# grantjr1842/delayed-streams-modeling

Measured on AMD Instinct MI355X. Metric: real-time stream throughput, stt-1b-en_fr @ bs=64 per GPU (Mimi encode + LM decode per 80 ms frame), higher is better.
Workload: dtype bf16 weights + bf16 KV, f32 activations as three exact bf16 pieces, f32 accumulate (v_mfma_f32_16x16x32_bf16); 1 GPU; stt-1b-en_fr batch=64 streaming, ring KV cache full (750 frames), Mimi encode + LM decode HIP path; streams_per_gpu=64, parallelism=replicas x1 (independent stream batches, no per-step collective), streams=encoder stream || 2 LM group stream(s)

## Files before the change

delayed-streams-modeling_amd/csrc/dsm_device.h:

```cpp
#pragma once
#include <hip/hip_runtime.h>

#include <atomic>
#include <cstdarg>
#include <cstdio>
#include <cstdlib>
#include <deque>
#include <mutex>
#include <shared_mutex>
#include <string>
#include <vector>

#include "../../include/dsm.h"
#include "dsm_gemm_plan.h"

#define HIPCHK_E(eng, expr)                                                                         \
  do {                                                                                              \
    hipError_t _e = (expr);                                                                         \
    if (_e != hipSuccess) {                                                                         \
      (eng)->set_error("%s failed: %s (%s:%d)", #expr, hipGetErrorString(_e), __FILE__, __LINE__);  \
      return DSM_ERR_DEVICE;                                                                        \
    }                                                                                               \
  } while (0)
#define HIPCHK(expr) HIPCHK_E(e, expr)

static void dsm_read_env(struct DsmDevice* e, bool stt);

struct DsmDevice {
  int device = 0;
  bool opened = false;
  hipStream_t s_enc = nullptr, s_model = nullptr;
  static constexpr int kMaxGroups = 4;
  hipStream_t s_grp[kMaxGroups] = {nullptr, nullptr, nullptr, nullptr};
  hipEvent_t ev_fork = nullptr, ev_grp_done[kMaxGroups] = {};
  bool prio_streams = false;
  int prio_hi = 0;
  bool use_graphs = true;
  bool fuse_qkv = true;
  bool stream_prio = false;
  bool fuse_front = true;
  int chunk_loop_min_tiles = GemmKnobs().chunk_loop_min_tiles;
  int loop_depth = GemmKnobs().loop_depth;
  int smallk_min_tiles = GemmKnobs().smallk_min_tiles;
  int smallk_mt = GemmKnobs().smallk_mt;
  size_t attn_lds_pad = 60000;
  int dot_mode = 0;

  int open(int device_id, int dot_mode_, bool stt) {
    device = device_id;
    dot_mode = dot_mode_;
    int ndev = 0;
    if (hipGetDeviceCount(&ndev) != hipSuccess || ndev <= device_id) {
      set_error("no usable HIP device %d (found %d): libdsm_mi355x has no CPU fallback", device_id, ndev);
      return DSM_ERR_DEVICE;
    }
    HIPCHK_E(this, hipSetDevice(device_id));
    opened = true;
    dsm_read_env(this, stt);
    prio_streams = stt;
    int prio_lo = 0;
    if (stt && stream_prio) (void)hipDeviceGetStreamPriorityRange(&prio_lo, &prio_hi);
    if (int rc = new_stream(&s_enc, prio_lo)) return rc;
    return new_stream(&s_model, prio_hi);
  }
  int new_stream(hipStream_t* out, int prio) {
    HIPCHK_E(this, prio_streams ? hipStreamCreateWithPriority(out, hipStreamNonBlocking, prio)
                                : hipStreamCreateWithFlags(out, hipStreamNonBlocking));
    return 0;
  }
  int open_groups(int G) {
    for (int g = 1; g < G; ++g) {
      if (int rc = new_stream(&s_grp[g], prio_hi)) return rc;
      if (int rc = new_event(&ev_grp_done[g])) return rc;
// ... 246 lines not shown
```

delayed-streams-modeling_amd/csrc/dsm_engine.hip:

```cpp
#include <hip/hip_runtime.h>

#include <cmath>
#include <cstdarg>
#include <cstdio>
#include <cstdlib>
#include <cstring>
#include <atomic>
#include <map>
#include <mutex>
#include <shared_mutex>
#include <string>
#include <set>
#include <vector>

#include "../../include/dsm.h"
#include "dsm_device.h"
#include "dsm_config_presets.h"
#include "dsm_gemm_plan.h"
#include "dsm_kernels.h"
#include "dsm_pcm_table.inc"
#include "dsm_numerics.h"
#include "dsm_safetensors.h"
#include "dsm_slot_blob.h"
#include "dsm_tts_slot_blob.h"
#include "dsm_tts_slot_layout.h"
#include "dsm_spm.h"
#include "dsm_slot_xfer.inc"
#include "dsm_asr_clip.h"

static thread_local std::string g_create_error;

static int dsm_env_int(const char* name, int dflt) {
  const char* v = getenv(name);
  return v ? atoi(v) : dflt;
}
static void dsm_read_env(DsmDevice* e, bool stt) {
  e->chunk_loop_min_tiles = gemm_default_knobs(stt, e->dot_mode).chunk_loop_min_tiles;
  if (stt && e->dot_mode == 1) e->attn_lds_pad = 40000;
  e->use_graphs = dsm_env_int("DSM_GRAPHS", 1) != 0;
  e->fuse_qkv = dsm_env_int("DSM_FUSE_QKV", 1) != 0;
  e->stream_prio = dsm_env_int("DSM_STREAM_PRIO", 0) != 0;
  e->fuse_front = dsm_env_int("DSM_FUSE_FRONT", 1) != 0;
  e->chunk_loop_min_tiles = dsm_env_int("DSM_CHUNK_LOOP_MIN", e->chunk_loop_min_tiles);
  e->loop_depth = dsm_env_int("DSM_LOOP_DEPTH", e->loop_depth) == 2 ? 2 : 4;
  e->smallk_min_tiles = dsm_env_int("DSM_SMALLK_MIN", e->smallk_min_tiles);
  const int mt = dsm_env_int("DSM_SMALLK_MT", e->smallk_mt);
  if (mt == 1 || mt == 2 || mt == 4) e->smallk_mt = mt;
}


namespace {

struct Linear {
  void* w = nullptr;
  float* bias = nullptr;
  int N = 0, K = 0, Npad = 0, Kpad = 0;
  bool bf16 = false;
  bool packed = false;
};

struct ConvGeom {
  Linear lin;
  int in_c = 0, out_c = 0, k = 0, stride = 1;
  int S = 0;
  int T_in = 0;
  int T_out = 0;
  bool replicate = false;
};

ConvGeom over_frames(const ConvGeom& g, int r) {
  ConvGeom c = g;
  c.T_in *= r;
  c.T_out *= r;
  return c;
}
// ... 1031 lines not shown
```

delayed-streams-modeling_amd/csrc/dsm_engine_api.inc:

```

namespace {

template <typename KVT, int HD, int T>
int launch_attn_t(DsmDevice* e, hipStream_t st, float* out, const float* q, const void* k, const void* v,
                  const uint32_t* start_pos, const uint8_t* active, int B, int H, int ctx, int d, const AttnFused& fq) {
  constexpr int UNR = (sizeof(KVT) == 2 && T == 1 && HD == 128) ? 8 : 4;
  size_t lds = sizeof(float) * ((size_t)T * ctx + 4 * T * HD + 16);
  if ((long)B * H >= 2048 && (size_t)2 * ctx * HD * sizeof(KVT) >= (size_t)256 * 1024) lds += e->attn_lds_pad;
  if (lds > 64 * 1024) {
    static size_t allowed = 0;
    if (lds > allowed) {
      HIPCHK(hipFuncSetAttribute(reinterpret_cast<const void*>(&attn_kernel<KVT, HD, T, UNR>), hipFuncAttributeMaxDynamicSharedMemorySize, (int)lds));
      allowed = lds;
    }
  }
  const int tag = e->tag_attn[e->sid(st)];
  if (T == 1 && HD == 64 && ctx <= 32) {
    const int ph = e->prof_begin(tag, st);
    hipLaunchKernelGGL((attn_small_kernel<KVT, 64>), dim3((B * H + 3) / 4), dim3(256), 0, st, out, q, reinterpret_cast<const KVT*>(k),
                       reinterpret_cast<const KVT*>(v), start_pos, active, B * H, H, ctx, d, fq);
    e->prof_end(ph, st);
    HIPCHK(hipGetLastError());
    return 0;
  }
// ... 123 lines not shown
    if (phase == 1) return 0;
    if (int rc = transformer_layer_tail<WT, KVT>(e, st, w, l, act, B, T, final_out, final_map, post_norm_w, post_norm_out, ca)) return rc;
  }
  return 0;
}

template <typename F>
int with_kv_type(bool kv_bf16, F&& f) {
  return kv_bf16 ? f(uint16_t{}) : f(float{});
}

int fork_groups(DsmDevice* e, hipStream_t st, size_t G) {
  if (G > 1) {
    HIPCHK(hipEventRecord(e->ev_fork, st));
    for (size_t g = 1; g < G; ++g) HIPCHK(hipStreamWaitEvent(e->s_grp[g], e->ev_fork, 0));
  }
  return 0;
}
template <typename F>
int run_groups(DsmDevice* e, hipStream_t st, size_t G, bool serialize, F&& body) {
  for (size_t g = G; g-- > 0;) {
    hipStream_t gs = (g == 0 || serialize) ? st : e->s_grp[g];
    if (int rc = body(g, gs)) return rc;
    if (g > 0) HIPCHK(hipEventRecord(e->ev_grp_done[g], gs));
  }
  return 0;
}
int join_groups(DsmDevice* e, hipStream_t st, size_t G) {
  for (size_t g = 1; g < G; ++g) HIPCHK(hipStreamWaitEvent(st, e->ev_grp_done[g], 0));
  return 0;
}

int seanet_encode(DsmDevice* e, hipStream_t st, const MimiW& w, SeanetEnc& s, const float* cat_init, int B, int r, float* out,
                  RowMap omap, bool front_done = false) {
  const RowMap none = plain_map(1, 1);
  const size_t n = w.stages.size();
  const ConvGeom g0 = over_frames(w.init_conv, r), gf = over_frames(w.final_conv, r);
  if (!front_done)
    if (int rc = run_conv(e, st, g0, cat_init, B, s.stages[0].y, plain_map(B * g0.T_out, g0.out_c), s.stages[0].cat_ra,
                          cat_map(over_frames(w.stages[0].ra, r)), nullptr, none))
      return rc;
  for (size_t i = 0; i < n; ++i) {
    const ConvGeom ra = over_frames(w.stages[i].ra, r), rb = over_frames(w.stages[i].rb, r), dn = over_frames(w.stages[i].down, r);
    SeanetEnc::Stage& ss = s.stages[i];
    if (!(i == 0 && front_done)) {
      if (int rc = run_conv(e, st, ra, ss.cat_ra, B, nullptr, none, ss.cat_rb, cat_map(rb), nullptr, none)) return rc;
      if (int rc = run_conv(e, st, rb, ss.cat_rb, B, nullptr, none, ss.cat_down, cat_map(dn), ss.y, plain_map(B * rb.T_out, rb.out_c)))
        return rc;
    }
    if (i + 1 < n) {
      if (int rc = run_conv(e, st, dn, ss.cat_down, B, s.stages[i + 1].y, plain_map(B * dn.T_out, dn.out_c), s.stages[i + 1].cat_ra,
                            cat_map(over_frames(w.stages[i + 1].ra, r)), nullptr, none))
        return rc;
    } else if (int rc = run_conv(e, st, dn, ss.cat_down, B, nullptr, none, s.cat_final, cat_map(gf), nullptr, none)) {
      return rc;
    }
  }
  return run_conv(e, st, gf, s.cat_final, B, out, omap, nullptr, none, nullptr, none);
}

int mimi_encode_body(dsm_engine* e, int side, hipStream_t st);
int mimi_encode(dsm_engine* e, int side, hipStream_t st) {
  return run_captured(e, *e->g_enc[side], st, (uint64_t)e->sid(st), [&] { return mimi_encode_body(e, side, st); });
}
int mimi_encode_body(dsm_engine* e, int side, hipStream_t st) {
  const MimiW& w = e->mimi_w;
  MimiState& s = e->mimi[side];
  const int B = e->B;
  const RowMap none = plain_map(1, 1);
  e->tag_gemm[e->sid(st)] = DSM_PROF_GEMM_MIMI;
  e->tag_attn[e->sid(st)] = DSM_PROF_ATTN_MIMI;
  bool fused_front = false;
  {
    const MimiW::Stage& s0 = w.stages[0];
    const ConvGeom& c = w.init_conv;
    fused_front = e->fuse_front && c.in_c == 1 && c.k == 7 && c.stride == 1 && c.out_c == 64 && c.S == 6 && !c.lin.bf16 &&
                  s0.ra.k == 3 && s0.ra.stride == 1 && s0.ra.in_c == 64 && s0.ra.out_c == 32 && s0.ra.S == 2 && !s0.ra.lin.bf16 &&
                  s0.rb.k == 1 && s0.rb.stride == 1 && s0.rb.in_c == 32 && s0.rb.out_c == 64 && !s0.rb.lin.bf16 &&
                  c.T_in % 64 == 0 && c.T_out == c.T_in && s0.ra.T_in == c.T_in && s0.rb.T_in == c.T_in && s0.down.in_c == 64 &&
                  s0.down.T_in == c.T_in && !c.replicate && !s0.ra.replicate;
    if (fused_front) {
      SeanetFrontArgs fa;
      fa.cat_init = s.enc.cat_init;
      fa.w0 = reinterpret_cast<const float*>(c.lin.w); fa.b0 = c.lin.bias; fa.ld0 = c.lin.Kpad;
      fa.w1 = reinterpret_cast<const float*>(s0.ra.lin.w); fa.b1 = s0.ra.lin.bias; fa.ld1 = s0.ra.lin.Kpad;
      fa.w2 = reinterpret_cast<const float*>(s0.rb.lin.w); fa.b2 = s0.rb.lin.bias; fa.ld2 = s0.rb.lin.Kpad;
      fa.cat_ra = s.enc.stages[0].cat_ra;
      fa.cat_down = s.enc.stages[0].cat_down;
      fa.T = c.T_in; fa.S0 = c.S; fa.Sd = s0.down.S;
      const int ph = e->prof_begin(e->tag_gemm[e->sid(st)], st);
      hipLaunchKernelGGL(seanet_front_kernel<64>, dim3(c.T_in / 64, B), dim3(256), seanet_front_lds<64>(), st, fa);
      e->prof_end(ph, st);
      HIPCHK(hipGetLastError());
    }
  }
  const int Tt = w.final_conv.T_out, d = w.cfg.dimension;
  if (int rc = seanet_encode(e, st, w, s.enc, s.enc.cat_init, B, 1, s.act.x, plain_map(B * Tt, d), fused_front)) return rc;
  if (int rc = transformer_forward<float, float>(e, st, w.tr, s.tr, s.act, B, Tt, s.mask, s.cat_ds, cat_map(w.downsample))) return rc;
  if (s.first_call && w.downsample.S > 0) {
    hipLaunchKernelGGL(conv_replicate_init_kernel, dim3(B), dim3(256), 0, st, s.h_descs[s.ds_desc], (const uint8_t*)s.keep);
    HIPCHK(hipGetLastError());
  }
  if (int rc = run_conv(e, st, w.downsample, s.cat_ds, B, s.latent, plain_map(B, d), nullptr, none, nullptr, none)) return rc;
  const int n_q = w.cfg.quantizer_n_q, qd = w.cfg.quantizer_dim;
  e->tag_gemm[e->sid(st)] = DSM_PROF_RVQ;
  for (int which = 0; which < 2; ++which) {
    const RvqW& r = which == 0 ? w.rvq_first : w.rvq_rest;
    if (r.n_q == 0) continue;
    float* res = which == 0 ? s.res_first : s.res_rest;
    {
      GemmArgs a = base_args(r.input_proj, s.latent, plain_map(B, d), B);
      a.Y = res; a.ymap = plain_map(B, qd);
      if (int rc = gemm_store<float>(e, st, a)) return rc;
    }
    for (int i = 0; i < r.n_q; ++i) {
      const Linear& cb = r.codebooks[i];
      GemmArgs a = base_args(cb, res, plain_map(B, qd), B);
      a.pval = s.pval; a.pidx = s.pidx;
      if (int rc = launch_gemm<float, float, EPI_RVQ, 1>(e, st, a, true)) return rc;
      hipLaunchKernelGGL(rvq_select_kernel, dim3(B), dim3(256), 0, st, s.pval, s.pidx, (cb.N + 15) / 16, B, s.codes, n_q,
                         which == 0 ? 0 : 1 + i, res, reinterpret_cast<const float*>(cb.w), qd, cb.Kpad);
      HIPCHK(hipGetLastError());
    }
  }
  if (!s.h_descs.empty()) {
    hipLaunchKernelGGL(conv_state_shift_kernel, dim3(B, (unsigned)s.h_descs.size()), dim3(256), 0, st, s.descs, s.mask,
                       s.first_call ? 1 : 0, nullptr, (const uint8_t*)(s.first_call ? s.keep : nullptr));
    HIPCHK(hipGetLastError());
  }
  s.first_call = false;
// ... 1309 lines not shown
    hipLaunchKernelGGL(fill_u32_kernel, dim3(g), dim3(256), 0, e->s_model, s.idx, pos % (uint32_t)ctx, (long)e->B);
  };
  fill(e->lm.tr, lm_pos, e->cfg.lm.context);
  for (int side = 0; side < 2; ++side)
    if (side == 0 || e->mimi1_ready.load(std::memory_order_acquire)) fill(e->mimi[side].tr, mimi_pos, e->cfg.mimi.transformer.context);
  HIPCHK(hipGetLastError());
  return dsm_sync(e);
}

int dsm_debug_set_text_tokens(dsm_engine* e, const uint32_t* tokens) {
  if (!e || !tokens) return DSM_ERR_INVALID;
  HIPCHK(hipSetDevice(e->device));
  ApiShared api(e);
  if (int rc = dsm_sync(e)) return rc;
  HIPCHK(hipMemcpy(e->lm.text_token, tokens, sizeof(uint32_t) * (size_t)e->B, hipMemcpyHostToDevice));
  return dsm_sync(e);
}

int dsm_debug_read(dsm_engine* e, const char* name, float* out, size_t cap) {
  if (!e || !name || !out) return DSM_ERR_INVALID;
  HIPCHK(hipSetDevice(e->device));
  ApiShared api(e);
  if (int rc = dsm_sync(e)) return rc;
  const float* src = nullptr;
  size_t n = 0;
  const int B = e->B, dim = e->cfg.mimi.dimension;
  int side = 0;
  std::string nm(name);
  if (nm.rfind("mimi1.", 0) == 0) { side = 1; nm = nm.substr(6); }
  else if (nm.rfind("mimi.", 0) == 0) nm = nm.substr(5);
  if (nm == "lm.hidden") { src = e->lm.hidden; n = (size_t)B * e->cfg.lm.d_model; }
  else if (nm == "lm.logits") { src = e->lm.logits; n = (size_t)B * e->cfg.text_out_vocab_size; }
  else if (nm == "latent") { src = e->mimi[side].latent; n = (size_t)B * dim; }
  if (!src) { e->set_error("unknown debug tap %s", name); return DSM_ERR_INVALID; }
  if (n > cap) n = cap;
  HIPCHK(hipMemcpy(out, src, sizeof(float) * n, hipMemcpyDeviceToHost));
  return (int)n;
}

int dsm_debug_gemm_plan(int stt, int dot_mode, int weight_bf16, int epi, int nt, int M, int N, int K, int flags, char* buf, size_t cap) {
  const int knobs[5] = {dot_mode, -1, -1, -1, -1};
  return dsm_debug_gemm_plan_knobs(stt, knobs, weight_bf16, epi, nt, M, N, K, flags, buf, cap);
}

}

namespace {
bool debug_knobs(const int* knobs, GemmKnobs* k) {
  if (knobs[0] >= 0) k->dot_mode = knobs[0];
  if (knobs[1] >= 0) k->chunk_loop_min_tiles = knobs[1];
  if (knobs[2] >= 0) k->smallk_min_tiles = knobs[2];
  if (knobs[3] >= 0) k->smallk_mt = knobs[3];
  if (knobs[4] >= 0) k->loop_depth = knobs[4];
  return (k->dot_mode == 0 || k->dot_mode == 1) && (k->smallk_mt == 1 || k->smallk_mt == 2 || k->smallk_mt == 4) &&
         (k->loop_depth == 2 || k->loop_depth == 4);
}

__global__ __launch_bounds__(256) void debug_slab_sum_kernel(float* Y, RowMap ymap, Slabs s, int M, int N) {
  const long i = (long)blockIdx.x * 256 + threadIdx.x;
  const int n4 = N >> 2;
  if (i >= (long)M * n4) return;
  const int m = (int)(i / n4), n = (int)(i % n4) * 4;
  const f32x4 v = slab_sum(s.ws + (long)m * s.ld + n, s.cstride, s.chunks);
  float* y = Y + ymap.off(m) + n;
  y[0] = v[0]; y[1] = v[1]; y[2] = v[2]; y[3] = v[3];
}
// ... 170 lines not shown
```

delayed-streams-modeling_amd/csrc/dsm_kernels.h:

```cpp
#pragma once
#include <hip/hip_runtime.h>
#include <stdint.h>
#include "dsm_numerics.h"
#include "dsm_sampling.h"
#include "dsm_token_scores.h"
#include "dsm_text_bias.h"
#include "dsm_pcm_format.h"

typedef float f32x4 __attribute__((ext_vector_type(4)));
typedef short dsm_bf16x8 __attribute__((ext_vector_type(8)));

__device__ __forceinline__ float wave_sum64(float v) {
#pragma unroll
  for (int off = 32; off >= 1; off >>= 1) v = v + __shfl_xor(v, off, 64);
  return v;
}

enum { EPI_STORE = 0, EPI_QKV = 1, EPI_GATE = 2, EPI_RVQ = 3 };

struct RowMap {
  long bstride;
  int rpb;
  int ld;
  int toff;
// ... 2139 lines not shown
      for (int i = 0; i < 4; ++i) o[i] = dsm_elu(a.b1 ? acc[m2][i] + a.b1[n + i] : acc[m2][i]);
      *reinterpret_cast<float4*>(&hs[m * C1 + 4 * ((n >> 2) ^ dsm_xs_sw(m))]) = make_float4(o[0], o[1], o[2], o[3]);
    }
  }
  __syncthreads();
  {
    f32x4 acc[MTILES];
#pragma unroll
    for (int mt = 0; mt < MTILES; ++mt) acc[mt] = (f32x4){0.f, 0.f, 0.f, 0.f};
    float wa[8], xb[MTILES][8];
    load_w8<float>(a.w2 + (long)(16 * wave + r) * a.ld2 + 8 * q, wa);
    const int xu0 = 4 * ((2 * q) ^ dsm_xs_sw(r)), xu1 = xu0 ^ 4;
#pragma unroll
    for (int mt = 0; mt < MTILES; ++mt) {
      const float* fp = &hs[(16 * mt + r) * C1];
      const float4 f0 = *reinterpret_cast<const float4*>(fp + xu0), f1 = *reinterpret_cast<const float4*>(fp + xu1);
      xb[mt][0] = f0.x; xb[mt][1] = f0.y; xb[mt][2] = f0.z; xb[mt][3] = f0.w;
      xb[mt][4] = f1.x; xb[mt][5] = f1.y; xb[mt][6] = f1.z; xb[mt][7] = f1.w;
    }
#pragma unroll
    for (int sidx = 0; sidx < 8; ++sidx)
#pragma unroll
      for (int mt = 0; mt < MTILES; ++mt) acc[mt] = __builtin_amdgcn_mfma_f32_16x16x4f32(wa[sidx], xb[mt][sidx], acc[mt], 0, 0, 0);
    float* out = a.cat_down + ((long)b * (a.Sd + a.T) + a.Sd + t0) * C0;
#pragma unroll
    for (int mt = 0; mt < MTILES; ++mt) {
      const int m = 16 * mt + r, n = 16 * wave + 4 * q;
      const float4 rv = *reinterpret_cast<const float4*>(&y0[m * C0 + 4 * ((n >> 2) ^ (m & 15))]);
      float o[4];
#pragma unroll
      for (int i = 0; i < 4; ++i) o[i] = a.b2 ? acc[mt][i] + a.b2[n + i] : acc[mt][i];
      o[0] = rv.x + o[0]; o[1] = rv.y + o[1]; o[2] = rv.z + o[2]; o[3] = rv.w + o[3];
      *reinterpret_cast<float4*>(out + (long)m * C0 + n) = make_float4(dsm_elu(o[0]), dsm_elu(o[1]), dsm_elu(o[2]), dsm_elu(o[3]));
    }
  }
}

struct ConvStateDesc {
  float* cat;
  long bstride;
  int S, T, C, replicate;
};

__global__ void conv_state_shift_kernel(const ConvStateDesc* __restrict__ descs, const uint8_t* __restrict__ active,
                                        int first_call, uint8_t* __restrict__ started, const uint8_t* __restrict__ keep) {
  const ConvStateDesc dsc = descs[blockIdx.y];
  const int b = blockIdx.x;
  float* base = dsc.cat + (long)b * dsc.bstride;
  const int n = dsc.S * dsc.C;
  if (active[b]) {
    const float* src = base + (long)dsc.T * dsc.C;
    for (int i = threadIdx.x; i < n; i += blockDim.x) base[i] = src[i];
    if (started && blockIdx.y == 0 && threadIdx.x == 0) started[b] = 1;
  } else if (first_call && !started && !(keep && keep[b])) {
    for (int i = threadIdx.x; i < n; i += blockDim.x) base[i] = 0.0f;
  }
}

__global__ void conv_replicate_init_kernel(ConvStateDesc dsc, const uint8_t* __restrict__ keep) {
  const int b = blockIdx.x;
  if (keep && keep[b]) return;
  float* base = dsc.cat + (long)b * dsc.bstride;
  const float* first = base + (long)dsc.S * dsc.C;
  for (int i = threadIdx.x; i < dsc.S * dsc.C; i += blockDim.x) base[i] = first[i % dsc.C];
}

// ... 665 lines not shown
```

Measured before the change: 1892 x realtime (stream-seconds of audio per wall second).

## Fuse SEANet stage-0 downsample and stage-1 residual block into one kernel

Adds seanet_stage1_kernel, which computes the stage-0 strided downsample conv, the stage-1 k=3 residual conv and the k=1 conv with the ELU and skip add in one launch. Each workgroup keeps a 30-frame tile plus halo in LDS and writes straight into the stage-1 down-conv input buffer. This removes three separate conv launches and the global round trips of their intermediates in the Mimi encoder. In exchange it recomputes the halo frames, depends on hard-coded channel and stride shapes guarded by a runtime check, and turns fuse_front into a tri-state so the path can be switched off.

```diff
diff --git a/delayed-streams-modeling_amd/csrc/dsm_device.h b/delayed-streams-modeling_amd/csrc/dsm_device.h
--- a/delayed-streams-modeling_amd/csrc/dsm_device.h
+++ b/delayed-streams-modeling_amd/csrc/dsm_device.h
@@ -38,7 +38,7 @@
   bool use_graphs = true;
   bool fuse_qkv = true;
   bool stream_prio = false;
-  bool fuse_front = true;
+  int fuse_front = 1;
   int chunk_loop_min_tiles = GemmKnobs().chunk_loop_min_tiles;
   int loop_depth = GemmKnobs().loop_depth;
   int smallk_min_tiles = GemmKnobs().smallk_min_tiles;
diff --git a/delayed-streams-modeling_amd/csrc/dsm_engine.hip b/delayed-streams-modeling_amd/csrc/dsm_engine.hip
--- a/delayed-streams-modeling_amd/csrc/dsm_engine.hip
+++ b/delayed-streams-modeling_amd/csrc/dsm_engine.hip
@@ -40,7 +40,8 @@
   e->use_graphs = dsm_env_int("DSM_GRAPHS", 1) != 0;
   e->fuse_qkv = dsm_env_int("DSM_FUSE_QKV", 1) != 0;
   e->stream_prio = dsm_env_int("DSM_STREAM_PRIO", 0) != 0;
-  e->fuse_front = dsm_env_int("DSM_FUSE_FRONT", 1) != 0;
+  e->fuse_front = dsm_env_int("DSM_FUSE_FRONT", 1);
+  if (e->fuse_front < 0 || e->fuse_front > 2) e->fuse_front = 1;
   e->chunk_loop_min_tiles = dsm_env_int("DSM_CHUNK_LOOP_MIN", e->chunk_loop_min_tiles);
   e->loop_depth = dsm_env_int("DSM_LOOP_DEPTH", e->loop_depth) == 2 ? 2 : 4;
   e->smallk_min_tiles = dsm_env_int("DSM_SMALLK_MIN", e->smallk_min_tiles);
diff --git a/delayed-streams-modeling_amd/csrc/dsm_engine_api.inc b/delayed-streams-modeling_amd/csrc/dsm_engine_api.inc
--- a/delayed-streams-modeling_amd/csrc/dsm_engine_api.inc
+++ b/delayed-streams-modeling_amd/csrc/dsm_engine_api.inc
@@ -179,7 +179,7 @@
 }
 
 int seanet_encode(DsmDevice* e, hipStream_t st, const MimiW& w, SeanetEnc& s, const float* cat_init, int B, int r, float* out,
-                  RowMap omap, bool front_done = false) {
+                  RowMap omap, bool front_done = false, const SeanetStage1Args* st1 = nullptr) {
   const RowMap none = plain_map(1, 1);
   const size_t n = w.stages.size();
   const ConvGeom g0 = over_frames(w.init_conv, r), gf = over_frames(w.final_conv, r);
@@ -190,12 +190,17 @@
   for (size_t i = 0; i < n; ++i) {
     const ConvGeom ra = over_frames(w.stages[i].ra, r), rb = over_frames(w.stages[i].rb, r), dn = over_frames(w.stages[i].down, r);
     SeanetEnc::Stage& ss = s.stages[i];
-    if (!(i == 0 && front_done)) {
+    if (!(i == 0 && front_done) && !(i == 1 && st1)) {
       if (int rc = run_conv(e, st, ra, ss.cat_ra, B, nullptr, none, ss.cat_rb, cat_map(rb), nullptr, none)) return rc;
       if (int rc = run_conv(e, st, rb, ss.cat_rb, B, nullptr, none, ss.cat_down, cat_map(dn), ss.y, plain_map(B * rb.T_out, rb.out_c)))
         return rc;
     }
-    if (i + 1 < n) {
+    if (i == 0 && st1) {
+      const int ph = e->prof_begin(e->tag_gemm[e->sid(st)], st);
+      hipLaunchKernelGGL(seanet_stage1_kernel, dim3(st1->T / kSeanetStage1Frames, B), dim3(256), seanet_stage1_lds(), st, *st1);
+      e->prof_end(ph, st);
+      HIPCHK(hipGetLastError());
+    } else if (i + 1 < n) {
       if (int rc = run_conv(e, st, dn, ss.cat_down, B, s.stages[i + 1].y, plain_map(B * dn.T_out, dn.out_c), s.stages[i + 1].cat_ra,
                             cat_map(over_frames(w.stages[i + 1].ra, r)), nullptr, none))
         return rc;
@@ -241,8 +246,30 @@
       HIPCHK(hipGetLastError());
     }
   }
+  SeanetStage1Args sa;
+  bool fused_stage1 = false;
+  if (e->fuse_front == 1 && w.stages.size() >= 2) {
+    const ConvGeom& dn = w.stages[0].down;
+    const MimiW::Stage& s1 = w.stages[1];
+    const int T = dn.T_out;
+    fused_stage1 = dn.in_c == 64 && dn.out_c == 128 && dn.k == 8 && dn.stride == 4 && dn.S == 4 && dn.T_in == 4 * T && !dn.lin.bf16 &&
+                   !dn.replicate && s1.ra.k == 3 && s1.ra.stride == 1 && s1.ra.in_c == 128 && s1.ra.out_c == 64 && s1.ra.S == 2 &&
+                   !s1.ra.lin.bf16 && !s1.ra.replicate && s1.rb.k == 1 && s1.rb.stride == 1 && s1.rb.in_c == 64 && s1.rb.out_c == 128 &&
+                   s1.rb.S == 0 && !s1.rb.lin.bf16 && T > 0 && T % kSeanetStage1Frames == 0 && s1.ra.T_in == T && s1.ra.T_out == T &&
+                   s1.rb.T_in == T && s1.rb.T_out == T && s1.down.in_c == 128 && s1.down.T_in == T;
+    if (fused_stage1) {
+      sa.cat_in = s.enc.stages[0].cat_down;
+      sa.wd = reinterpret_cast<const float*>(dn.lin.w); sa.bd = dn.lin.bias; sa.ldd = dn.lin.Kpad;
+      sa.w1 = reinterpret_cast<const float*>(s1.ra.lin.w); sa.b1 = s1.ra.lin.bias; sa.ld1 = s1.ra.lin.Kpad;
+      sa.w2 = reinterpret_cast<const float*>(s1.rb.lin.w); sa.b2 = s1.rb.lin.bias; sa.ld2 = s1.rb.lin.Kpad;
+      sa.cat_ra = s.enc.stages[1].cat_ra;
+      sa.cat_down = s.enc.stages[1].cat_down;
+      sa.T = T; sa.S0 = dn.S; sa.Sd = s1.down.S;
+    }
+  }
   const int Tt = w.final_conv.T_out, d = w.cfg.dimension;
-  if (int rc = seanet_encode(e, st, w, s.enc, s.enc.cat_init, B, 1, s.act.x, plain_map(B * Tt, d), fused_front)) return rc;
+  if (int rc = seanet_encode(e, st, w, s.enc, s.enc.cat_init, B, 1, s.act.x, plain_map(B * Tt, d), fused_front, fused_stage1 ? &sa : nullptr))
+    return rc;
   if (int rc = transformer_forward<float, float>(e, st, w.tr, s.tr, s.act, B, Tt, s.mask, s.cat_ds, cat_map(w.downsample))) return rc;
   if (s.first_call && w.downsample.S > 0) {
     hipLaunchKernelGGL(conv_replicate_init_kernel, dim3(B), dim3(256), 0, st, s.h_descs[s.ds_desc], (const uint8_t*)s.keep);
diff --git a/delayed-streams-modeling_amd/csrc/dsm_kernels.h b/delayed-streams-modeling_amd/csrc/dsm_kernels.h
--- a/delayed-streams-modeling_amd/csrc/dsm_kernels.h
+++ b/delayed-streams-modeling_amd/csrc/dsm_kernels.h
@@ -2195,6 +2195,229 @@
       for (int i = 0; i < 4; ++i) o[i] = a.b2 ? acc[mt][i] + a.b2[n + i] : acc[mt][i];
       o[0] = rv.x + o[0]; o[1] = rv.y + o[1]; o[2] = rv.z + o[2]; o[3] = rv.w + o[3];
       *reinterpret_cast<float4*>(out + (long)m * C0 + n) = make_float4(dsm_elu(o[0]), dsm_elu(o[1]), dsm_elu(o[2]), dsm_elu(o[3]));
+    }
+  }
+}
+
+struct SeanetStage1Args {
+  const float* cat_in;
+  const float *wd, *bd;
+  const float *w1, *b1;
+  const float *w2, *b2;
+  float* cat_ra;
+  float* cat_down;
+  int ldd, ld1, ld2;
+  int T, S0, Sd;
+};
+
+constexpr int kSeanetStage1Frames = 30;
+constexpr size_t seanet_stage1_lds() { return sizeof(float) * (132 * 64); }
+static_assert(4 * seanet_stage1_lds() <= 160 * 1024 && 34 * 128 + 32 * 64 <= 132 * 64, "four workgroups per CU; e1 and hs fit the input region");
+
+__global__ __launch_bounds__(256) void seanet_stage1_kernel(SeanetStage1Args a) {
+  constexpr int CI = 64, C1 = 128, CH = 64, TF = kSeanetStage1Frames, RIN = 4 * 32 + 4;
+  constexpr int PF = 2;
+  extern __shared__ __attribute__((aligned(16))) float st1_lds[];
+  float* xin = st1_lds;
+  float* e1 = xin;
+  float* hs = e1 + 34 * C1;
+  const int tid = threadIdx.x, lane = tid & 63, wave = tid >> 6;
+  const int r = lane & 15, q = lane >> 4;
+  const int b = blockIdx.y, t0 = blockIdx.x * TF;
+  const bool first = t0 == 0, last = t0 + TF == a.T;
+
+  const float* wrow0 = a.wd + (long)(32 * wave + r) * a.ldd + 8 * q;
+  const float* wrow1 = wrow0 + (long)16 * a.ldd;
+  float wa[PF + 1][2][8];
+#pragma unroll
+  for (int p = 0; p < PF; ++p) {
+    load_w8<float>(wrow0 + 32 * p, wa[p][0]);
+    load_w8<float>(wrow1 + 32 * p, wa[p][1]);
+  }
+  {
+    const float* src = a.cat_in + (long)b * (a.S0 + 4 * a.T) * CI;
+    constexpr int PIECES = RIN * (CI / 4), PER = (PIECES + 255) / 256;
+    float4 v[PER];
+#pragma unroll
+    for (int j = 0; j < PER; ++j) {
+      const int i = min(tid + 256 * j, PIECES - 1);
+      const int g = max(4 * (t0 - 2) + (i >> 4), 0);
+      v[j] = *reinterpret_cast<const float4*>(src + (long)g * CI + 4 * (i & 15));
+    }
+#pragma unroll
+    for (int j = 0; j < PER; ++j) {
+      const int i = tid + 256 * j, p = i >> 4;
+      if (i < PIECES) *reinterpret_cast<float4*>(&xin[p * CI + 4 * ((i & 15) ^ ((p >> 2) & 15))]) = v[j];
+    }
+  }
+  __syncthreads();
+  f32x4 y1[2][2];
+  {
+    f32x4 acc[2][2], tot[2][2];
+#pragma unroll
+    for (int blk = 0; blk < 16; ++blk) {
+      if ((blk & 7) == 0) {
+#pragma unroll
+        for (int nt = 0; nt < 2; ++nt)
+#pragma unroll
+          for (int mt = 0; mt < 2; ++mt) acc[nt][mt] = (f32x4){0.f, 0.f, 0.f, 0.f};
+      }
+      if (blk + PF < 16) {
+        load_w8<float>(wrow0 + 32 * (blk + PF), wa[(blk + PF) % (PF + 1)][0]);
+        load_w8<float>(wrow1 + 32 * (blk + PF), wa[(blk + PF) % (PF + 1)][1]);
+      }
+      const int tap = blk >> 1, u0 = (blk & 1) * 8 + 2 * q;
+      float xb[2][8];
+#pragma unroll
+      for (int mt = 0; mt < 2; ++mt) {
+        const int p = 4 * (16 * mt + r) + tap, sw = (p >> 2) & 15;
+        const float4 f0 = *reinterpret_cast<const float4*>(&xin[p * CI + 4 * (u0 ^ sw)]);
+        const float4 f1 = *reinterpret_cast<const float4*>(&xin[p * CI + 4 * ((u0 + 1) ^ sw)]);
+        xb[mt][0] = f0.x; xb[mt][1] = f0.y; xb[mt][2] = f0.z; xb[mt][3] = f0.w;
+        xb[mt][4] = f1.x; xb[mt][5] = f1.y; xb[mt][6] = f1.z; xb[mt][7] = f1.w;
+      }
+      const int wb = blk % (PF + 1);
+#pragma unroll
+      for (int sidx = 0; sidx < 8; ++sidx)
+#pragma unroll
+        for (int nt = 0; nt < 2; ++nt)
+#pragma unroll
+          for (int mt = 0; mt < 2; ++mt) acc[nt][mt] = __builtin_amdgcn_mfma_f32_16x16x4f32(wa[wb][nt][sidx], xb[mt][sidx], acc[nt][mt], 0, 0, 0);
+      if ((blk & 7) == 7) {
+#pragma unroll
+        for (int nt = 0; nt < 2; ++nt)
+#pragma unroll
+          for (int mt = 0; mt < 2; ++mt)
+#pragma unroll
+            for (int i = 0; i < 4; ++i) tot[nt][mt][i] = blk == 7 ? acc[nt][mt][i] : dsm_unpaired(tot[nt][mt][i] + acc[nt][mt][i]);
+      }
+    }
+    const float* w1row = a.w1 + (long)(16 * wave + r) * a.ld1 + 8 * q;
+#pragma unroll
+    for (int p = 0; p < PF; ++p) load_w8<float>(w1row + 32 * p, wa[p][0]);
+    __syncthreads();
+#pragma unroll
+    for (int nt = 0; nt < 2; ++nt) {
+      const int n = 32 * wave + 16 * nt + 4 * q;
+      float bv[4] = {0.f, 0.f, 0.f, 0.f};
+      if (a.bd) {
+        const float4 t = *reinterpret_cast<const float4*>(a.bd + n);
+        bv[0] = t.x; bv[1] = t.y; bv[2] = t.z; bv[3] = t.w;
+      }
+#pragma unroll
+      for (int mt = 0; mt < 2; ++mt) {
+        const int R = 16 * mt + r;
+#pragma unroll
+        for (int i = 0; i < 4; ++i) y1[nt][mt][i] = a.bd ? dsm_unpaired(tot[nt][mt][i] + bv[i]) : tot[nt][mt][i];
+        float4 ev = make_float4(dsm_elu(y1[nt][mt][0]), dsm_elu(y1[nt][mt][1]), dsm_elu(y1[nt][mt][2]), dsm_elu(y1[nt][mt][3]));
+        if (first && R < 2) ev = *reinterpret_cast<const float4*>(a.cat_ra + ((long)b * (2 + a.T) + R) * C1 + n);
+        if (last && R >= TF)
+          *reinterpret_cast<float4*>(a.cat_ra + ((long)b * (2 + a.T) + 2 + (t0 - 2 + R)) * C1 + n) = ev;
+        *reinterpret_cast<float4*>(&e1[(R + 2) * C1 + 4 * ((n >> 2) ^ ((R + 2) & 15))]) = ev;
+      }
+    }
+  }
+  __syncthreads();
+  {
+    const float* w1row = a.w1 + (long)(16 * wave + r) * a.ld1 + 8 * q;
+    f32x4 acc[2], tot[2];
+#pragma unroll
+    for (int blk = 0; blk < 12; ++blk) {
+      if ((blk & 7) == 0) {
+#pragma unroll
+        for (int mt = 0; mt < 2; ++mt) acc[mt] = (f32x4){0.f, 0.f, 0.f, 0.f};
+      }
+      if (blk + PF < 12) load_w8<float>(w1row + 32 * (blk + PF), wa[(blk + PF) % (PF + 1)][0]);
+      const int tap = blk >> 2, u0 = (blk & 3) * 8 + 2 * q;
+      float xb[2][8];
+#pragma unroll
+      for (int mt = 0; mt < 2; ++mt) {
+        const int s = 16 * mt + r + tap, sw = s & 15;
+        const float4 f0 = *reinterpret_cast<const float4*>(&e1[s * C1 + 4 * (u0 ^ sw)]);
+        const float4 f1 = *reinterpret_cast<const float4*>(&e1[s * C1 + 4 * ((u0 + 1) ^ sw)]);
+        xb[mt][0] = f0.x; xb[mt][1] = f0.y; xb[mt][2] = f0.z; xb[mt][3] = f0.w;
+        xb[mt][4] = f1.x; xb[mt][5] = f1.y; xb[mt][6] = f1.z; xb[mt][7] = f1.w;
+      }
+      const int wb = blk % (PF + 1);
+#pragma unroll
+      for (int sidx = 0; sidx < 8; ++sidx)
+#pragma unroll
+        for (int mt = 0; mt < 2; ++mt) acc[mt] = __builtin_amdgcn_mfma_f32_16x16x4f32(wa[wb][0][sidx], xb[mt][sidx], acc[mt], 0, 0, 0);
+      if (blk == 7 || blk == 11) {
+#pragma unroll
+        for (int mt = 0; mt < 2; ++mt)
+#pragma unroll
+          for (int i = 0; i < 4; ++i) tot[mt][i] = blk == 7 ? acc[mt][i] : dsm_unpaired(tot[mt][i] + acc[mt][i]);
+      }
+    }
+    const int n = 16 * wave + 4 * q;
+    float bv[4] = {0.f, 0.f, 0.f, 0.f};
+    if (a.b1) {
+      const float4 t = *reinterpret_cast<const float4*>(a.b1 + n);
+      bv[0] = t.x; bv[1] = t.y; bv[2] = t.z; bv[3] = t.w;
+    }
+#pragma unroll
+    for (int mt = 0; mt < 2; ++mt) {
+      const int R = 16 * mt + r;
+      float o[4];
+#pragma unroll
+      for (int i = 0; i < 4; ++i) o[i] = dsm_elu(a.b1 ? dsm_unpaired(tot[mt][i] + bv[i]) : tot[mt][i]);
+      *reinterpret_cast<float4*>(&hs[R * CH + 4 * ((n >> 2) ^ (R & 15))]) = make_float4(o[0], o[1], o[2], o[3]);
+    }
+  }
+  {
+    const float* w2row = a.w2 + (long)(32 * wave + r) * a.ld2 + 8 * q;
+    float wc[2][2][8];
+#pragma unroll
+    for (int blk = 0; blk < 2; ++blk) {
+      load_w8<float>(w2row + 32 * blk, wc[blk][0]);
+      load_w8<float>(w2row + (long)16 * a.ld2 + 32 * blk, wc[blk][1]);
+    }
+    __syncthreads();
+    f32x4 acc[2][2];
+#pragma unroll
+    for (int nt = 0; nt < 2; ++nt)
+#pragma unroll
+      for (int mt = 0; mt < 2; ++mt) acc[nt][mt] = (f32x4){0.f, 0.f, 0.f, 0.f};
+#pragma unroll
+    for (int blk = 0; blk < 2; ++blk) {
+      const int u0 = blk * 8 + 2 * q;
+      float xb[2][8];
+#pragma unroll
+      for (int mt = 0; mt < 2; ++mt) {
+        const int R = 16 * mt + r, sw = R & 15;
+        const float4 f0 = *reinterpret_cast<const float4*>(&hs[R * CH + 4 * (u0 ^ sw)]);
+        const float4 f1 = *reinterpret_cast<const float4*>(&hs[R * CH + 4 * ((u0 + 1) ^ sw)]);
+        xb[mt][0] = f0.x; xb[mt][1] = f0.y; xb[mt][2] = f0.z; xb[mt][3] = f0.w;
+        xb[mt][4] = f1.x; xb[mt][5] = f1.y; xb[mt][6] = f1.z; xb[mt][7] = f1.w;
+      }
+#pragma unroll
+      for (int sidx = 0; sidx < 8; ++sidx)
+#pragma unroll
+        for (int nt = 0; nt < 2; ++nt)
+#pragma unroll
+          for (int mt = 0; mt < 2; ++mt) acc[nt][mt] = __builtin_amdgcn_mfma_f32_16x16x4f32(wc[blk][nt][sidx], xb[mt][sidx], acc[nt][mt], 0, 0, 0);
+    }
+    float* out = a.cat_down + ((long)b * (a.Sd + a.T) + a.Sd + t0 - 2) * C1;
+#pragma unroll
+    for (int nt = 0; nt < 2; ++nt) {
+      const int n = 32 * wave + 16 * nt + 4 * q;
+      float bv[4] = {0.f, 0.f, 0.f, 0.f};
+      if (a.b2) {
+        const float4 t = *reinterpret_cast<const float4*>(a.b2 + n);
+        bv[0] = t.x; bv[1] = t.y; bv[2] = t.z; bv[3] = t.w;
+      }
+#pragma unroll
+      for (int mt = 0; mt < 2; ++mt) {
+        const int R = 16 * mt + r;
+        float o[4];
+#pragma unroll
+        for (int i = 0; i < 4; ++i) {
+          const float t = a.b2 ? dsm_unpaired(acc[nt][mt][i] + bv[i]) : acc[nt][mt][i];
+          o[i] = dsm_elu(dsm_unpaired(y1[nt][mt][i] + t));
+        }
+        if (R >= 2) *reinterpret_cast<float4*>(out + (long)R * C1 + n) = make_float4(o[0], o[1], o[2], o[3]);
+      }
     }
   }
 }
```

After: 1876 x realtime (stream-seconds of audio per wall second). Within noise of the previous version (-0.8%).

## Fuse SEANet stage-0 downsample conv into the fused front kernel

Applied to the files above, without the earlier changes.

Adds seanet_front_down_kernel, which extends the existing fused init-conv/residual-block front kernel to also compute the stride-4 downsample conv into stage-1 y and cat_ra, keeping the stage-0 output tile in LDS. It uses a 4-frame halo, recomputed per tile, so the separate downsample launch and its round trip of the cat_down activation through global memory can be skipped. The kernel is gated by shape checks and an env flag that defaults on, and debug taps are added for checking. The cost is more LDS per block, redundant halo compute, and split-K accumulation that may change summation order slightly.

```diff
diff --git a/delayed-streams-modeling_amd/csrc/dsm_device.h b/delayed-streams-modeling_amd/csrc/dsm_device.h
--- a/delayed-streams-modeling_amd/csrc/dsm_device.h
+++ b/delayed-streams-modeling_amd/csrc/dsm_device.h
@@ -39,6 +39,7 @@
   bool fuse_qkv = true;
   bool stream_prio = false;
   bool fuse_front = true;
+  bool fuse_down = true;
   int chunk_loop_min_tiles = GemmKnobs().chunk_loop_min_tiles;
   int loop_depth = GemmKnobs().loop_depth;
   int smallk_min_tiles = GemmKnobs().smallk_min_tiles;
diff --git a/delayed-streams-modeling_amd/csrc/dsm_engine.hip b/delayed-streams-modeling_amd/csrc/dsm_engine.hip
--- a/delayed-streams-modeling_amd/csrc/dsm_engine.hip
+++ b/delayed-streams-modeling_amd/csrc/dsm_engine.hip
@@ -41,6 +41,7 @@
   e->fuse_qkv = dsm_env_int("DSM_FUSE_QKV", 1) != 0;
   e->stream_prio = dsm_env_int("DSM_STREAM_PRIO", 0) != 0;
   e->fuse_front = dsm_env_int("DSM_FUSE_FRONT", 1) != 0;
+  e->fuse_down = dsm_env_int("DSM_FUSE_DOWN", 1) != 0;
   e->chunk_loop_min_tiles = dsm_env_int("DSM_CHUNK_LOOP_MIN", e->chunk_loop_min_tiles);
   e->loop_depth = dsm_env_int("DSM_LOOP_DEPTH", e->loop_depth) == 2 ? 2 : 4;
   e->smallk_min_tiles = dsm_env_int("DSM_SMALLK_MIN", e->smallk_min_tiles);
diff --git a/delayed-streams-modeling_amd/csrc/dsm_engine_api.inc b/delayed-streams-modeling_amd/csrc/dsm_engine_api.inc
--- a/delayed-streams-modeling_amd/csrc/dsm_engine_api.inc
+++ b/delayed-streams-modeling_amd/csrc/dsm_engine_api.inc
@@ -179,7 +179,7 @@
 }
 
 int seanet_encode(DsmDevice* e, hipStream_t st, const MimiW& w, SeanetEnc& s, const float* cat_init, int B, int r, float* out,
-                  RowMap omap, bool front_done = false) {
+                  RowMap omap, bool front_done = false, bool down0_done = false) {
   const RowMap none = plain_map(1, 1);
   const size_t n = w.stages.size();
   const ConvGeom g0 = over_frames(w.init_conv, r), gf = over_frames(w.final_conv, r);
@@ -195,6 +195,7 @@
       if (int rc = run_conv(e, st, rb, ss.cat_rb, B, nullptr, none, ss.cat_down, cat_map(dn), ss.y, plain_map(B * rb.T_out, rb.out_c)))
         return rc;
     }
+    if (i == 0 && down0_done) continue;
     if (i + 1 < n) {
       if (int rc = run_conv(e, st, dn, ss.cat_down, B, s.stages[i + 1].y, plain_map(B * dn.T_out, dn.out_c), s.stages[i + 1].cat_ra,
                             cat_map(over_frames(w.stages[i + 1].ra, r)), nullptr, none))
@@ -217,7 +218,7 @@
   const RowMap none = plain_map(1, 1);
   e->tag_gemm[e->sid(st)] = DSM_PROF_GEMM_MIMI;
   e->tag_attn[e->sid(st)] = DSM_PROF_ATTN_MIMI;
-  bool fused_front = false;
+  bool fused_front = false, fused_down = false;
   {
     const MimiW::Stage& s0 = w.stages[0];
     const ConvGeom& c = w.init_conv;
@@ -226,6 +227,10 @@
                   s0.rb.k == 1 && s0.rb.stride == 1 && s0.rb.in_c == 32 && s0.rb.out_c == 64 && !s0.rb.lin.bf16 &&
                   c.T_in % 64 == 0 && c.T_out == c.T_in && s0.ra.T_in == c.T_in && s0.rb.T_in == c.T_in && s0.down.in_c == 64 &&
                   s0.down.T_in == c.T_in && !c.replicate && !s0.ra.replicate;
+    const ConvGeom& dn = s0.down;
+    fused_down = fused_front && e->fuse_down && w.stages.size() > 1 && dn.out_c == 128 && dn.k == 8 && dn.stride == 4 && dn.S == 4 &&
+                 !dn.lin.bf16 && dn.lin.Kpad == 512 && dn.T_out * 4 == dn.T_in && !dn.replicate && w.stages[1].ra.in_c == 128 &&
+                 w.stages[1].ra.T_in == dn.T_out && !w.stages[1].ra.replicate;
     if (fused_front) {
       SeanetFrontArgs fa;
       fa.cat_init = s.enc.cat_init;
@@ -236,13 +241,23 @@
       fa.cat_down = s.enc.stages[0].cat_down;
       fa.T = c.T_in; fa.S0 = c.S; fa.Sd = s0.down.S;
       const int ph = e->prof_begin(e->tag_gemm[e->sid(st)], st);
-      hipLaunchKernelGGL(seanet_front_kernel<64>, dim3(c.T_in / 64, B), dim3(256), seanet_front_lds<64>(), st, fa);
+      if (fused_down) {
+        SeanetFrontDownArgs fd;
+        fd.f = fa;
+        fd.wd = reinterpret_cast<const float*>(dn.lin.w); fd.bd = dn.lin.bias; fd.ldd = dn.lin.Kpad;
+        fd.y1 = s.enc.stages[1].y;
+        fd.cat_ra1 = s.enc.stages[1].cat_ra;
+        fd.S1 = w.stages[1].ra.S;
+        hipLaunchKernelGGL(seanet_front_down_kernel<64>, dim3(c.T_in / 64, B), dim3(256), seanet_front_down_lds<64>(), st, fd);
+      } else {
+        hipLaunchKernelGGL(seanet_front_kernel<64>, dim3(c.T_in / 64, B), dim3(256), seanet_front_lds<64>(), st, fa);
+      }
       e->prof_end(ph, st);
       HIPCHK(hipGetLastError());
     }
   }
   const int Tt = w.final_conv.T_out, d = w.cfg.dimension;
-  if (int rc = seanet_encode(e, st, w, s.enc, s.enc.cat_init, B, 1, s.act.x, plain_map(B * Tt, d), fused_front)) return rc;
+  if (int rc = seanet_encode(e, st, w, s.enc, s.enc.cat_init, B, 1, s.act.x, plain_map(B * Tt, d), fused_front, fused_down)) return rc;
   if (int rc = transformer_forward<float, float>(e, st, w.tr, s.tr, s.act, B, Tt, s.mask, s.cat_ds, cat_map(w.downsample))) return rc;
   if (s.first_call && w.downsample.S > 0) {
     hipLaunchKernelGGL(conv_replicate_init_kernel, dim3(B), dim3(256), 0, st, s.h_descs[s.ds_desc], (const uint8_t*)s.keep);
@@ -1618,6 +1633,20 @@
   if (nm == "lm.hidden") { src = e->lm.hidden; n = (size_t)B * e->cfg.lm.d_model; }
   else if (nm == "lm.logits") { src = e->lm.logits; n = (size_t)B * e->cfg.text_out_vocab_size; }
   else if (nm == "latent") { src = e->mimi[side].latent; n = (size_t)B * dim; }
+  else if (e->mimi_w.stages.size() > 1 && (nm == "seanet.s1.y" || nm == "seanet.s1.cat_ra" || nm == "seanet.s0.cat_down_tail")) {
+    const MimiW::Stage& s0 = e->mimi_w.stages[0];
+    const MimiW::Stage& s1 = e->mimi_w.stages[1];
+    const SeanetEnc& enc = e->mimi[side].enc;
+    if (nm == "seanet.s1.y") { src = enc.stages[1].y; n = (size_t)B * s1.ra.T_in * s1.ra.in_c; }
+    else if (nm == "seanet.s1.cat_ra") { src = enc.stages[1].cat_ra; n = (size_t)B * (s1.ra.S + s1.ra.T_in) * s1.ra.in_c; }
+    else {
+      n = (size_t)s0.down.S * s0.down.in_c;
+      if ((size_t)B * n > cap) { e->set_error("debug tap %s needs %zu floats", name, (size_t)B * n); return DSM_ERR_INVALID; }
+      HIPCHK(hipMemcpy2D(out, sizeof(float) * n, enc.stages[0].cat_down + (size_t)s0.down.T_in * s0.down.in_c, sizeof(float) * (s0.down.S + s0.down.T_in) * s0.down.in_c,
+                         sizeof(float) * n, B, hipMemcpyDeviceToHost));
+      return (int)(B * n);
+    }
+  }
   if (!src) { e->set_error("unknown debug tap %s", name); return DSM_ERR_INVALID; }
   if (n > cap) n = cap;
   HIPCHK(hipMemcpy(out, src, sizeof(float) * n, hipMemcpyDeviceToHost));
diff --git a/delayed-streams-modeling_amd/csrc/dsm_kernels.h b/delayed-streams-modeling_amd/csrc/dsm_kernels.h
--- a/delayed-streams-modeling_amd/csrc/dsm_kernels.h
+++ b/delayed-streams-modeling_amd/csrc/dsm_kernels.h
@@ -2195,6 +2195,206 @@
       for (int i = 0; i < 4; ++i) o[i] = a.b2 ? acc[mt][i] + a.b2[n + i] : acc[mt][i];
       o[0] = rv.x + o[0]; o[1] = rv.y + o[1]; o[2] = rv.z + o[2]; o[3] = rv.w + o[3];
       *reinterpret_cast<float4*>(out + (long)m * C0 + n) = make_float4(dsm_elu(o[0]), dsm_elu(o[1]), dsm_elu(o[2]), dsm_elu(o[3]));
+    }
+  }
+}
+
+struct SeanetFrontDownArgs {
+  SeanetFrontArgs f;
+  const float *wd, *bd;
+  float* y1;
+  float* cat_ra1;
+  int ldd, S1;
+};
+
+__device__ __forceinline__ int fd_sw(int row) { return ((row >> 2) ^ ((row & 3) << 2)) & 15; }
+
+template <int TM>
+constexpr size_t seanet_front_down_lds() { return sizeof(float) * ((TM + 18) * 64 + (TM + 16) * 64 + (TM + 16) * 32 + (TM + 16)); }
+template <int TM>
+__global__ __launch_bounds__(256) void seanet_front_down_kernel(SeanetFrontDownArgs fa) {
+  constexpr int C0 = 64, C1 = 32, C2 = 128, TAPS0 = 7, HALO = 4, F = TM + HALO, MTILES = TM / 16 + 1, ROWS = 16 * MTILES;
+  static_assert(TM == 64, "tile");
+  const SeanetFrontArgs& a = fa.f;
+  extern __shared__ __attribute__((aligned(16))) float front_down_lds[];
+  float* e0 = front_down_lds;
+  float* y0 = e0 + (ROWS + 2) * C0;
+  float* hs = y0 + ROWS * C0;
+  float* xs = hs + ROWS * C1;
+  float* ot = e0;
+  const int tid = threadIdx.x, lane = tid & 63, wave = __builtin_amdgcn_readfirstlane(tid >> 6);
+  const int r = lane & 15, q = lane >> 4;
+  const int b = blockIdx.y, t0 = blockIdx.x * TM;
+  const bool first = t0 == 0, last = t0 + TM == a.T;
+  const float* cat = a.cat_init + (long)b * (a.S0 + a.T);
+  for (int i = tid; i < F + 2 + TAPS0 - 1; i += 256) {
+    const int c = t0 - 6 + i;
+    xs[i] = c >= 0 ? cat[c] : 0.0f;
+  }
+  const int cq = tid & 15;
+  float w0r[4][TAPS0], b0r[4];
+#pragma unroll
+  for (int j = 0; j < 4; ++j) {
+#pragma unroll
+    for (int sidx = 0; sidx < TAPS0; ++sidx) w0r[j][sidx] = a.w0[(long)(4 * cq + j) * a.ld0 + sidx];
+    b0r[j] = a.b0 ? a.b0[4 * cq + j] : 0.0f;
+  }
+  __syncthreads();
+  for (int R = tid >> 4; R < F + 2; R += 16) {
+    float4 ev;
+    if (first && R < 6) {
+      ev = R >= 4 ? *reinterpret_cast<const float4*>(a.cat_ra + ((long)b * (2 + a.T) + (R - 4)) * C0 + 4 * cq) : make_float4(0.f, 0.f, 0.f, 0.f);
+    } else {
+      float xr[TAPS0];
+#pragma unroll
+      for (int sidx = 0; sidx < TAPS0; ++sidx) xr[sidx] = xs[R + sidx];
+      float yv[4];
+#pragma unroll
+      for (int j = 0; j < 4; ++j) {
+        float acc = 0.0f;
+#pragma unroll
+        for (int sidx = 0; sidx < TAPS0; ++sidx) acc = dsm_unpaired(DSM_FMAF(w0r[j][sidx], xr[sidx], acc));
+        yv[j] = a.b0 ? dsm_unpaired(acc + b0r[j]) : acc;
+      }
+      ev = make_float4(dsm_elu(yv[0]), dsm_elu(yv[1]), dsm_elu(yv[2]), dsm_elu(yv[3]));
+      if (R >= 2) *reinterpret_cast<float4*>(&y0[(R - 2) * C0 + 4 * (cq ^ ((R - 2) & 15))]) = make_float4(yv[0], yv[1], yv[2], yv[3]);
+      if (last && R >= F)
+        *reinterpret_cast<float4*>(a.cat_ra + ((long)b * (2 + a.T) + 2 + (t0 - 6 + R)) * C0 + 4 * cq) = ev;
+    }
+    *reinterpret_cast<float4*>(&e0[R * C0 + 4 * (cq ^ (R & 15))]) = ev;
+  }
+  __syncthreads();
+  {
+    const int nt = wave & 1, mh = wave >> 1;
+    const bool fifth = mh == 0;
+    f32x4 acc[3];
+#pragma unroll
+    for (int m2 = 0; m2 < 3; ++m2) acc[m2] = (f32x4){0.f, 0.f, 0.f, 0.f};
+    const float* wrow = a.w1 + (long)(16 * nt + r) * a.ld1 + 8 * q;
+#pragma unroll
+    for (int blk = 0; blk < 6; ++blk) {
+      float wa[8], xb[3][8];
+      load_w8<float>(wrow + 32 * blk, wa);
+      const int tap = blk >> 1, u0 = (blk & 1) * 8 + 2 * q;
+#pragma unroll
+      for (int m2 = 0; m2 < 3; ++m2) {
+        const int R = 16 * (m2 < 2 ? 2 * mh + m2 : 4) + r + tap;
+        const float4 f0 = *reinterpret_cast<const float4*>(&e0[R * C0 + 4 * (u0 ^ (R & 15))]);
+        const float4 f1 = *reinterpret_cast<const float4*>(&e0[R * C0 + 4 * ((u0 + 1) ^ (R & 15))]);
+        xb[m2][0] = f0.x; xb[m2][1] = f0.y; xb[m2][2] = f0.z; xb[m2][3] = f0.w;
+        xb[m2][4] = f1.x; xb[m2][5] = f1.y; xb[m2][6] = f1.z; xb[m2][7] = f1.w;
+      }
+#pragma unroll
+      for (int sidx = 0; sidx < 8; ++sidx)
+#pragma unroll
+        for (int m2 = 0; m2 < 3; ++m2) acc[m2] = __builtin_amdgcn_mfma_f32_16x16x4f32(wa[sidx], xb[m2][sidx], acc[m2], 0, 0, 0);
+    }
+#pragma unroll
+    for (int m2 = 0; m2 < 3; ++m2) {
+      if (m2 == 2 && !fifth) continue;
+      const int m = 16 * (m2 < 2 ? 2 * mh + m2 : 4) + r, n = 16 * nt + 4 * q;
+      if (m >= F) continue;
+      float o[4];
+#pragma unroll
+      for (int i = 0; i < 4; ++i) o[i] = dsm_elu(a.b1 ? dsm_unpaired(acc[m2][i] + a.b1[n + i]) : acc[m2][i]);
+      *reinterpret_cast<float4*>(&hs[m * C1 + 4 * ((n >> 2) ^ dsm_xs_sw(m))]) = make_float4(o[0], o[1], o[2], o[3]);
+    }
+  }
+  __syncthreads();
+  Raw8<float> rw0[2], rw1[2];
+  const float* wdrow[2];
+#pragma unroll
+  for (int nt = 0; nt < 2; ++nt) wdrow[nt] = fa.wd + (long)(32 * wave + 16 * nt + r) * fa.ldd + 8 * q;
+  {
+    f32x4 acc[MTILES];
+#pragma unroll
+    for (int mt = 0; mt < MTILES; ++mt) acc[mt] = (f32x4){0.f, 0.f, 0.f, 0.f};
+    float wa[8], xb[MTILES][8];
+    load_w8<float>(a.w2 + (long)(16 * wave + r) * a.ld2 + 8 * q, wa);
+    const int xu0 = 4 * ((2 * q) ^ dsm_xs_sw(r)), xu1 = xu0 ^ 4;
+#pragma unroll
+    for (int mt = 0; mt < MTILES; ++mt) {
+      const float* fp = &hs[(16 * mt + r) * C1];
+      const float4 f0 = *reinterpret_cast<const float4*>(fp + xu0), f1 = *reinterpret_cast<const float4*>(fp + xu1);
+      xb[mt][0] = f0.x; xb[mt][1] = f0.y; xb[mt][2] = f0.z; xb[mt][3] = f0.w;
+      xb[mt][4] = f1.x; xb[mt][5] = f1.y; xb[mt][6] = f1.z; xb[mt][7] = f1.w;
+    }
+#pragma unroll
+    for (int sidx = 0; sidx < 8; ++sidx)
+#pragma unroll
+      for (int mt = 0; mt < MTILES; ++mt) acc[mt] = __builtin_amdgcn_mfma_f32_16x16x4f32(wa[sidx], xb[mt][sidx], acc[mt], 0, 0, 0);
+#pragma unroll
+    for (int nt = 0; nt < 2; ++nt) {
+      rw0[nt].load(wdrow[nt]);
+      rw1[nt].load(wdrow[nt] + 32);
+    }
+    float* cd = a.cat_down + (long)b * (a.Sd + a.T) * C0;
+#pragma unroll
+    for (int mt = 0; mt < MTILES; ++mt) {
+      const int m = 16 * mt + r, n = 16 * wave + 4 * q;
+      if (m >= F) continue;
+      float4 ov;
+      if (first && m < HALO) {
+        ov = *reinterpret_cast<const float4*>(cd + (long)m * C0 + n);
+      } else {
+        const float4 rv = *reinterpret_cast<const float4*>(&y0[m * C0 + 4 * ((n >> 2) ^ (m & 15))]);
+        float o[4];
+#pragma unroll
+        for (int i = 0; i < 4; ++i) o[i] = a.b2 ? dsm_unpaired(acc[mt][i] + a.b2[n + i]) : acc[mt][i];
+        o[0] = dsm_unpaired(rv.x + o[0]); o[1] = dsm_unpaired(rv.y + o[1]); o[2] = dsm_unpaired(rv.z + o[2]); o[3] = dsm_unpaired(rv.w + o[3]);
+        ov = make_float4(dsm_elu(o[0]), dsm_elu(o[1]), dsm_elu(o[2]), dsm_elu(o[3]));
+        if (last && m >= TM)
+          *reinterpret_cast<float4*>(cd + (long)(a.Sd + t0 - HALO + m) * C0 + n) = ov;
+      }
+      *reinterpret_cast<float4*>(&ot[m * C0 + 4 * ((n >> 2) ^ fd_sw(m))]) = ov;
+    }
+  }
+  __syncthreads();
+  {
+    f32x4 acc[2], tot[2];
+#pragma unroll
+    for (int nt = 0; nt < 2; ++nt) {
+      acc[nt] = (f32x4){0.f, 0.f, 0.f, 0.f};
+      tot[nt] = (f32x4){0.f, 0.f, 0.f, 0.f};
+    }
+#pragma unroll
+    for (int blk = 0; blk < 16; ++blk) {
+      float wa[2][8], xb[8];
+#pragma unroll
+      for (int nt = 0; nt < 2; ++nt) {
+        if (blk & 1) rw1[nt].unpack(wa[nt]); else rw0[nt].unpack(wa[nt]);
+        if (blk + 2 < 16) {
+          if (blk & 1) rw1[nt].load(wdrow[nt] + 32 * (blk + 2)); else rw0[nt].load(wdrow[nt] + 32 * (blk + 2));
+        }
+      }
+      const int tap = blk >> 1, u0 = (blk & 1) * 8 + 2 * q, R = 4 * r + tap;
+      const float4 f0 = *reinterpret_cast<const float4*>(&ot[R * C0 + 4 * (u0 ^ fd_sw(R))]);
+      const float4 f1 = *reinterpret_cast<const float4*>(&ot[R * C0 + 4 * ((u0 + 1) ^ fd_sw(R))]);
+      xb[0] = f0.x; xb[1] = f0.y; xb[2] = f0.z; xb[3] = f0.w;
+      xb[4] = f1.x; xb[5] = f1.y; xb[6] = f1.z; xb[7] = f1.w;
+#pragma unroll
+      for (int sidx = 0; sidx < 8; ++sidx)
+#pragma unroll
+        for (int nt = 0; nt < 2; ++nt) acc[nt] = __builtin_amdgcn_mfma_f32_16x16x4f32(wa[nt][sidx], xb[sidx], acc[nt], 0, 0, 0);
+      if ((blk & 7) == 7) {
+#pragma unroll
+        for (int nt = 0; nt < 2; ++nt) {
+#pragma unroll
+          for (int i = 0; i < 4; ++i) tot[nt][i] = dsm_unpaired(tot[nt][i] + acc[nt][i]);
+          acc[nt] = (f32x4){0.f, 0.f, 0.f, 0.f};
+        }
+      }
+    }
+    const int To = a.T / 4, mo = t0 / 4 + r;
+#pragma unroll
+    for (int nt = 0; nt < 2; ++nt) {
+      const int n = 32 * wave + 16 * nt + 4 * q;
+      float o[4];
+#pragma unroll
+      for (int i = 0; i < 4; ++i) o[i] = fa.bd ? dsm_unpaired(tot[nt][i] + fa.bd[n + i]) : tot[nt][i];
+      *reinterpret_cast<float4*>(fa.y1 + ((long)b * To + mo) * C2 + n) = make_float4(o[0], o[1], o[2], o[3]);
+      *reinterpret_cast<float4*>(fa.cat_ra1 + ((long)b * (fa.S1 + To) + fa.S1 + mo) * C2 + n) =
+          make_float4(dsm_elu(o[0]), dsm_elu(o[1]), dsm_elu(o[2]), dsm_elu(o[3]));
     }
   }
 }
```

Result: no change. 1858 x realtime (stream-seconds of audio per wall second) before, 1855 x realtime (stream-seconds of audio per wall second) after (-0.1%).
